# wzjin2017/fhe-fed

Measured on AMD Instinct MI355X. Metric: ciphertexts aggregated/sec (+ encode+enc / dec+decode ms), N clients, ring 2^15 L=4, higher is better.
Workload: dtype u64; 1 GPU; cfg3: 16 learners/GPU x ResNet-18 (11689512 params -> 714 cts of 16384 slots), ring 2^15, L=4 towers; ring_dim=32768, towers=4, learners_total=16, cts_per_learner=714, parallelism=dp1 (one GPU, no collective), layout=arena

## Files before the change

### fhe-fed_amd/csrc/eval.cpp

```cpp
#include <algorithm>
#include <cstring>
#include <fstream>
#include <sstream>

#include "api_util.h"
#include "palisade_codec.h"
#include "shelfi_internal.h"

namespace shelfi {

constexpr int kMaxDigits = 3;

struct LevelState {
  bool built = false;
  bool q_built = false;
  bool own_q = false;
  DeviceTables q;
  DeviceTables ext;
  DeviceTables dtf[kMaxDigits];
  uint64_t* ks = nullptr;
  KsArgs args{};
};

struct EvalState {
// ... 299 lines not shown
  K.T = p.L + ev.kP;
  K.dnum = ev.dnum;
  for (uint32_t t = 0; t < K.T; ++t) {
    K.q.push_back(t < p.L ? p.q[t] : ev.p[t - p.L]);
    K.psi.push_back(t < p.L ? p.psi[t] : ev.ppsi[t - p.L]);
  }
  for (auto& v : K.poly_versions) v = 0;
  return K;
}

static std::string slurp(const std::string& path) {
  std::ifstream f(path, std::ios::binary);
  if (!f) throw Error{SHELFI_ERR_IO, "cannot read " + path};
  std::ostringstream ss;
  ss << f.rdbuf();
  return ss.str();
}

static void load_evalkey(shelfi_ctx* ctx, const std::string& file) {
  EvalState& ev = eval_state(ctx);
  const PalisadeEvalKey K = palisade_parse_evalmult_key((const uint8_t*)file.data(), file.size());
  const Params& p = ctx->p;
  if (ctx->pal_keytag.empty() || K.keytag != ctx->pal_keytag)
    throw Error{SHELFI_ERR_FORMAT, "evaluation key belongs to another key pair (key tag)"};
  if (K.N != p.N || K.T != p.L + ev.kP || K.dnum != ev.dnum)
    throw Error{SHELFI_ERR_FORMAT, "evaluation key was made for other parameters"};
  for (uint32_t t = 0; t < K.T; ++t)
    if (K.q[t] != (t < p.L ? p.q[t] : ev.p[t - p.L]))
      throw Error{SHELFI_ERR_FORMAT, "evaluation key towers differ from this context's Q and special primes"};
  if (K.tower_off.size() != 2ull * K.dnum * K.T) throw Error{SHELFI_ERR_FORMAT, "evaluation key tower count"};
  for (uint32_t t = 0; t < K.T; ++t)
    if (K.psi[t] != (t < p.L ? p.psi[t] : ev.ppsi[t - p.L]))
      throw Error{SHELFI_ERR_FORMAT, "evaluation key roots of unity differ from this context's"};
  std::vector<uint64_t> polys(K.tower_off.size() * (size_t)K.N);
  for (size_t i = 0; i < K.tower_off.size(); ++i)
    std::memcpy(polys.data() + i * K.N, file.data() + K.tower_off[i], (size_t)K.N * 8);
  install_evk(ctx, ev, polys.data());
}

void load_evalkey_if_present(shelfi_ctx* ctx, const std::string& dir) {
  std::string file;
  try {
    file = slurp(dir + "key-eval-mult.txt");
  } catch (const Error&) {
    return;
  }
  try {
    load_evalkey(ctx, file);
  } catch (const Error&) {
  }
}

static uint64_t chunk_of(uint64_t K, size_t per_ct) {
  const uint64_t cap = std::max<uint64_t>(1, (2048ull << 20) / std::max<size_t>(per_ct, 1));
  const uint64_t n = (K + cap - 1) / cap;
  return n ? (K + n - 1) / n : 1;
}

}

using namespace shelfi;

extern "C" {

int shelfi_special_primes(uint32_t ring_dim, uint32_t num_towers, const uint64_t* moduli, uint32_t* dnum,
                          uint32_t* alpha, uint32_t* num_special, uint64_t* special, uint64_t* special_roots) {
  if (!moduli || !dnum || !alpha || !num_special || !special || num_towers < 1 ||
      num_towers > (uint32_t)kMaxTowers || ring_dim < 2 || (ring_dim & (ring_dim - 1)))
    return SHELFI_ERR_ARG;
  return guarded([&] {
    uint64_t p[kMaxTowers], r[kMaxTowers];
    special_primes(ring_dim, num_towers, moduli, dnum, alpha, num_special, p, r);
    for (uint32_t i = 0; i < *num_special; ++i) {
      special[i] = p[i];
      if (special_roots) special_roots[i] = r[i];
    }
  });
}

int shelfi_eval_key_info(const shelfi_ctx* ctx, uint32_t* dnum, uint32_t* alpha, uint32_t* num_special,
                         uint64_t* special, int* has_key) {
  if (!ctx || !dnum || !alpha || !num_special) return SHELFI_ERR_ARG;
  std::lock_guard<std::mutex> lk(ctx->mu);
  return guarded([&] {
    uint64_t p[kMaxTowers];
    special_primes(ctx->p.N, ctx->p.L, ctx->p.q, dnum, alpha, num_special, p, nullptr);
    if (special)
      for (uint32_t i = 0; i < *num_special; ++i) special[i] = p[i];
    if (has_key) *has_key = (ctx->ev && ctx->ev->evk) ? 1 : 0;
  });
}

size_t shelfi_eval_key_words(const shelfi_ctx* ctx) {
  if (!ctx) return 0;
  uint32_t dn, al, kP;
  uint64_t p[kMaxTowers];
  special_primes(ctx->p.N, ctx->p.L, ctx->p.q, &dn, &al, &kP, p, nullptr);
  return 2ull * dn * (ctx->p.L + kP) * ctx->p.N;
}

}

namespace shelfi {
static std::vector<uint64_t> switch_keygen(shelfi_ctx* ctx, uint32_t galois) {
  require_keys(ctx);
  const Params& p = ctx->p;
  EvalState& ev = eval_state(ctx);
// ... 360 lines not shown
```

### fhe-fed_amd/csrc/kernels.hip

```cpp
#include <hip/hip_runtime.h>

#include <algorithm>
#include <cmath>
#include <cstring>
#include <type_traits>
#include <vector>

#include "dev_common.h"
#include "shelfi_internal.h"

namespace shelfi {

static uint32_t xcd_combos(uint64_t G) {
  if (!switches().xcd_order) return 0;
  return (G % 8 == 0 && G <= 0xFFFFFFFFull) ? (uint32_t)G : 0;
}

template <int LOGR>
__global__ __launch_bounds__(256) void ntt_fwd_cols(uint64_t* __restrict__ polys, uint32_t L,
                                                    uint32_t logN, const uint64_t* __restrict__ tw,
                                                    const uint64_t* __restrict__ twp,
                                                    const TowerConst* __restrict__ tcs) {
  constexpr int R = 1 << LOGR;
  const uint32_t N = 1u << logN;
// ... 613 lines not shown
    return (uint32_t)n;
  }();
  uint64_t pc = (uint64_t)cus * per_cu / ncombo;
  if (pc < 1) pc = 1;
  if (pc > K) pc = K;
  return (uint32_t)pc;
}

template <class FZ = NoFuse>
__global__ __launch_bounds__(256) void ntt_inv_blocks(uint64_t* __restrict__ polys, uint32_t L,
                                                      uint32_t logN, uint32_t blkLog,
                                                      const uint64_t* __restrict__ tw,
                                                      const uint64_t* __restrict__ twp,
                                                      const TowerConst* __restrict__ tcs,
                                                      int scale_ninv,
                                                      const uint64_t* __restrict__ ct,
                                                      const uint64_t* __restrict__ sk,
                                                      const uint64_t* __restrict__ sksh, int sum_in,
                                                      uint32_t ctL, FZ fz) {
  constexpr bool FUSE = std::is_same<FZ, FuseIn>::value;
  extern __shared__ __attribute__((aligned(16))) uint64_t sm[];
  const uint32_t N = 1u << logN, blk = 1u << blkLog;
  const uint32_t sh = logN - blkLog, nb = 1u << sh;
  const uint64_t poly = blockIdx.x >> sh;
  const uint32_t b = blockIdx.x & (nb - 1);
  const uint32_t t = (uint32_t)(poly % L);
  const TowerConst& c = tcs[t];
  const uint64_t q = c.q;
  uint64_t* __restrict__ a = polys + poly * N + ((uint64_t)b << blkLog);
  if constexpr (FUSE) {
    const uint64_t e0 = ((poly / L) * ctL << logN) + ((uint64_t)t << logN) + ((uint64_t)b << blkLog);
    for (uint32_t p = threadIdx.x; p < blk / 2; p += 256) {
      ulonglong2 x = make_ulonglong2(0, 0);
      for (uint32_t i = 0; i < fz.P; ++i) {
        const ulonglong2 y = reinterpret_cast<const ulonglong2*>(fz.part[i] + e0)[p];
        x.x += y.x;
        x.y += y.y;
      }
      lds_put2(sm, p, make_ulonglong2(red64(x.x, q, c.one_shoup), red64(x.y, q, c.one_shoup)));
    }
  } else if (ct) {
    const uint64_t kk = poly / L, off = ((uint64_t)t << logN) + ((uint64_t)b << blkLog);
    const ulonglong2* c0 = reinterpret_cast<const ulonglong2*>(ct + (kk * 2 * ctL << logN) + off);
    const ulonglong2* c1 = reinterpret_cast<const ulonglong2*>(ct + ((kk * 2 + 1) * ctL << logN) + off);
    const ulonglong2* s = reinterpret_cast<const ulonglong2*>(sk + off);
    const ulonglong2* ss = reinterpret_cast<const ulonglong2*>(sksh + off);
    for (uint32_t p = threadIdx.x; p < blk / 2; p += 256) {
      ulonglong2 x0 = c0[p];
      const ulonglong2 x1 = c1[p], sv = s[p], sw = ss[p];
      if (sum_in) x0 = make_ulonglong2(red64(x0.x, q, c.one_shoup), red64(x0.y, q, c.one_shoup));
      lds_put2(sm, p, make_ulonglong2(addmod(x0.x, shoup_mul(x1.x, sv.x, sw.x, q), q),
                                      addmod(x0.y, shoup_mul(x1.y, sv.y, sw.y, q), q)));
    }
  } else {
    for (uint32_t p = threadIdx.x; p < blk / 2; p += 256)
      lds_put2(sm, p, reinterpret_cast<const ulonglong2*>(a)[p]);
  }
  __syncthreads();
  ntt_inv_block_stages(sm, blkLog, b, logN, tw + (uint64_t)t * N, twp + (uint64_t)t * N, q);
  if (scale_ninv) {
    const uint64_t ni = c.ninv, nip = c.ninv_shoup;
    for (uint32_t p = threadIdx.x; p < blk / 2; p += 256) {
      const ulonglong2 v = lds_get2(sm, p);
      reinterpret_cast<ulonglong2*>(a)[p] = make_ulonglong2(canon4(shoup_lazy(v.x, ni, nip, q), q),
                                                            canon4(shoup_lazy(v.y, ni, nip, q), q));
    }
  } else {
    for (uint32_t p = threadIdx.x; p < blk / 2; p += 256)
      reinterpret_cast<ulonglong2*>(a)[p] = lds_get2(sm, p);
  }
}

template <int LOGR>
__global__ __launch_bounds__(256) void ntt_inv_cols(uint64_t* __restrict__ polys, uint32_t L,
                                                    uint32_t logN, const uint64_t* __restrict__ tw,
                                                    const uint64_t* __restrict__ twp,
                                                    const TowerConst* __restrict__ tcs) {
  constexpr int R = 1 << LOGR;
  const uint32_t N = 1u << logN;
  const uint32_t BLK = N >> LOGR;
  const uint32_t bpp = BLK / 256;
  const uint64_t poly = blockIdx.x / bpp;
  const uint32_t col = (blockIdx.x % bpp) * 256 + threadIdx.x;
  const uint32_t t = (uint32_t)(poly % L);
  const TowerConst& c = tcs[t];
  const uint64_t q = c.q;
  const uint64_t* __restrict__ w = tw + (uint64_t)t * N;
  const uint64_t* __restrict__ wp = twp + (uint64_t)t * N;
  uint64_t* __restrict__ a = polys + poly * N + col;
  uint64_t x[R];
#pragma unroll
  for (int r = 0; r < R; ++r) x[r] = a[(uint64_t)r * BLK];
#pragma unroll
  for (int v = 0; v < LOGR; ++v) {
    const int tr = 1 << v, h = R >> (v + 1);
#pragma unroll
    for (int i = 0; i < h; ++i) {
      const uint64_t W = w[h + i], Wp = wp[h + i];
#pragma unroll
      for (int jj = 0; jj < tr; ++jj) {
        const int r0 = 2 * i * tr + jj, r1 = r0 + tr;
        if (gs_in8<true>(v, jj))
          gs_bfly_b<true>(x[r0], x[r1], W, Wp, q, c.n8q);
        else
          gs_bfly_b<false>(x[r0], x[r1], W, Wp, q, c.n8q);
      }
    }
  }
  const uint64_t ni = c.ninv, nip = c.ninv_shoup;
#pragma unroll
  for (int r = 0; r < R; ++r) a[(uint64_t)r * BLK] = canon4(shoup_lazy(x[r], ni, nip, q), q);
}

#define NTT_DISPATCH(LOGRV, KERNEL, ...)                                                   \
  switch (LOGRV) {                                                                       \
    case 1: hipLaunchKernelGGL(KERNEL<1>, __VA_ARGS__); break;                           \
    case 2: hipLaunchKernelGGL(KERNEL<2>, __VA_ARGS__); break;                           \
    case 3: hipLaunchKernelGGL(KERNEL<3>, __VA_ARGS__); break;                           \
    case 4: hipLaunchKernelGGL(KERNEL<4>, __VA_ARGS__); break;                           \
    case 5: hipLaunchKernelGGL(KERNEL<5>, __VA_ARGS__); break;                           \
    case 6: hipLaunchKernelGGL(KERNEL<6>, __VA_ARGS__); break;                           \
    default: throw Error{SHELFI_ERR_ARG, "unsupported ring dimension"};                  \
  }

template <int BL, int K1, int K2, int K3, int K4>
__global__ __launch_bounds__(256) void ntt_fwd_blocks_ct(uint64_t* polys, uint32_t L, uint32_t logN,
                                                         const ulonglong2* __restrict__ twb,
                                                         const TowerConst* __restrict__ tcs) {
  __shared__ __attribute__((aligned(16))) uint64_t sm[lpad_size(BL)];
  const uint32_t sh = logN - BL;
  const uint64_t poly = blockIdx.x >> sh;
  const uint32_t b = blockIdx.x & ((1u << sh) - 1);
  const uint32_t t = (uint32_t)(poly % L);
  const TowerConst& c = tcs[t];
  uint64_t* base = polys + (poly << logN) + ((uint64_t)b << BL);
  fwd_block_pass_ct<BL, K1, K2, K3, K4>(base, twb + ((uint64_t)t << logN) + ((uint64_t)b << BL), c.q, c.n8q, sm,
                                        [&](uint32_t j0, auto& x) {
#pragma unroll
                                          for (int m = 0; m < (1 << K4); m += 2)
                                            *reinterpret_cast<ulonglong2*>(base + j0 + m) =
                                                make_ulonglong2(red_any(x[m], c), red_any(x[m + 1], c));
                                        });
}
template <int BL, int K1, int K2, int K3, int K4>
__global__ __launch_bounds__(256) void ntt_inv_blocks_ct(uint64_t* polys, uint32_t L, uint32_t logN,
                                                         const ulonglong2* __restrict__ twb,
                                                         const TowerConst* __restrict__ tcs) {
  static_assert(K1 + K2 + K3 + K4 == BL, "chunk plan must cover the block");
  __shared__ __attribute__((aligned(16))) uint64_t sm[lpad_size(BL)];
  const uint32_t sh = logN - BL;
  const uint64_t poly = blockIdx.x >> sh;
  const uint32_t b = blockIdx.x & ((1u << sh) - 1);
  const uint32_t t = (uint32_t)(poly % L);
  const uint64_t q = tcs[t].q, n8q = tcs[t].n8q;
  uint64_t* base = polys + (poly << logN) + ((uint64_t)b << BL);
  const ulonglong2* __restrict__ tb = twb + ((uint64_t)t << logN) + ((uint64_t)b << BL);
  const auto lds_ld = [&](uint32_t, uint32_t pj) { return sm[pj]; };
  inv_chunk_ct<BL, 0, K1, false>(tb, q, n8q, [&](uint32_t j, uint32_t) { return base[j]; },
                                 [&](int, uint32_t, uint32_t pj0, auto& x) {
#pragma unroll
                                   for (int m = 0; m < (1 << K1); ++m) sm[pj0 + lofs<1>(m)] = x[m];
                                 });
  __syncthreads();
  inv_chunk_ct<BL, K1, K2, true>(tb, q, n8q, lds_ld, [&](int, uint32_t, uint32_t pj0, auto& x) {
#pragma unroll
    for (int m = 0; m < (1 << K2); ++m) sm[pj0 + lofs<(1 << K1)>(m)] = x[m];
  });
  __syncthreads();
  inv_chunk_ct<BL, K1 + K2, K3, true>(tb, q, n8q, lds_ld, [&](int, uint32_t, uint32_t pj0, auto& x) {
#pragma unroll
    for (int m = 0; m < (1 << K3); ++m) sm[pj0 + lofs<(1 << (K1 + K2))>(m)] = x[m];
  });
  __syncthreads();
  inv_chunk_ct<BL, BL - K4, K4, true>(tb, q, n8q, lds_ld, [&](int, uint32_t j0, uint32_t, auto& x) {
#pragma unroll
    for (int m = 0; m < (1 << K4); ++m) base[j0 + (m << (BL - K4))] = x[m];
  });
}

void launch_ntt(uint64_t* polys, uint64_t P, uint32_t L, uint32_t logN, bool inverse,
                const DeviceTables& dt, hipStream_t s) {
  if (!P) return;
  const uint32_t N = 1u << logN;
  const uint32_t blkLog = ntt_block_log(logN);
  const int logR = (int)(logN - blkLog);
  const uint32_t blk = 1u << blkLog;
  const size_t lds = (size_t)blk * sizeof(uint64_t);
  const uint64_t nbBlocks = P << logR;
  const uint64_t nbCols = P * ((N >> logR) / 256);
  if (nbBlocks > 0x7FFFFFFFull || nbCols > 0x7FFFFFFFull)
    throw Error{SHELFI_ERR_ARG, "NTT batch too large"};
  if (!inverse) {
    if (logR > 0) {
      NTT_DISPATCH(logR, ntt_fwd_cols, dim3((uint32_t)nbCols), dim3(256), 0, s, polys, L, logN,
                   dt.psi_rev, dt.psi_rev_sh, dt.tc);
    }
    if (logR > 0 && blkLog == 11 && dt.red_ok)
      hipLaunchKernelGGL((ntt_fwd_blocks_ct<11, 3, 3, 3, 2>), dim3((uint32_t)nbBlocks), dim3(256), 0, s, polys, L,
                         logN, dt.tw_fwd_blk, dt.tc);
    else if (logR > 0 && blkLog == 12 && dt.red_ok)
      hipLaunchKernelGGL((ntt_fwd_blocks_ct<12, 3, 3, 3, 3>), dim3((uint32_t)nbBlocks), dim3(256), 0, s, polys, L,
                         logN, dt.tw_fwd_blk, dt.tc);
    else
      hipLaunchKernelGGL(ntt_fwd_blocks, dim3((uint32_t)nbBlocks), dim3(256), lds, s, polys, L,
                         logN, (uint32_t)logR, dt.psi_rev, dt.psi_rev_sh, dt.tc);
  } else {
    if (logR > 0 && blkLog == 11 && dt.red_ok)
      hipLaunchKernelGGL((ntt_inv_blocks_ct<11, 2, 3, 3, 3>), dim3((uint32_t)nbBlocks), dim3(256), 0, s, polys, L,
                         logN, dt.tw_inv_blk, dt.tc);
    else if (logR > 0 && blkLog == 12 && dt.red_ok)
      hipLaunchKernelGGL((ntt_inv_blocks_ct<12, 3, 3, 3, 3>), dim3((uint32_t)nbBlocks), dim3(256), 0, s, polys, L,
                         logN, dt.tw_inv_blk, dt.tc);
    else
      hipLaunchKernelGGL(ntt_inv_blocks<>, dim3((uint32_t)nbBlocks), dim3(256), lds, s, polys, L,
                         logN, blkLog, dt.ipsi_rev, dt.ipsi_rev_sh, dt.tc, logR == 0 ? 1 : 0,
                         (const uint64_t*)nullptr, (const uint64_t*)nullptr, (const uint64_t*)nullptr, 0, L,
                         NoFuse{});
    if (logR > 0) {
      NTT_DISPATCH(logR, ntt_inv_cols, dim3((uint32_t)nbCols), dim3(256), 0, s, polys, L, logN,
                   dt.ipsi_rev, dt.ipsi_rev_sh, dt.tc);
    }
  }
  SHELFI_HIP(hipGetLastError());
}

void launch_ntt_cols(uint64_t* polys, uint64_t P, uint32_t L, uint32_t logN, bool inverse,
                     const DeviceTables& dt, hipStream_t s) {
  const uint32_t N = 1u << logN;
  const int logR = (int)(logN - ntt_block_log(logN));
  if (!P || logR == 0) return;
  const uint64_t nbCols = P * ((N >> logR) / 256);
  if (nbCols > 0x7FFFFFFFull) throw Error{SHELFI_ERR_ARG, "NTT batch too large"};
  if (!inverse)
    NTT_DISPATCH(logR, ntt_fwd_cols, dim3((uint32_t)nbCols), dim3(256), 0, s, polys, L, logN, dt.psi_rev,
                 dt.psi_rev_sh, dt.tc)
  else
    NTT_DISPATCH(logR, ntt_inv_cols, dim3((uint32_t)nbCols), dim3(256), 0, s, polys, L, logN, dt.ipsi_rev,
                 dt.ipsi_rev_sh, dt.tc)
  SHELFI_HIP(hipGetLastError());
}

template <int LOGR>
__global__ __launch_bounds__(256) void fft_inv_cols(const double* __restrict__ x, uint64_t n,
                                                    double2* __restrict__ buf, uint32_t logS,
                                                    const double2* __restrict__ tw) {
  constexpr int R = 1 << LOGR;
  const uint32_t S = 1u << logS;
  const uint32_t BLK = S >> LOGR;
  const uint32_t bpp = BLK / 256;
  const uint64_t k = blockIdx.x / bpp;
  const uint32_t col = (blockIdx.x % bpp) * 256 + threadIdx.x;
  double2 v[R];
#pragma unroll
  for (int r = 0; r < R; ++r) {
    const uint64_t gi = k * S + col + (uint64_t)r * BLK;
    v[r] = make_double2(gi < n ? x[gi] : 0.0, 0.0);
  }
#pragma unroll
  for (int s = 0; s < LOGR; ++s) {
    const uint32_t len = S >> s, lenh = len >> 1;
    const int trr = R >> (s + 1);
#pragma unroll
    for (int r0 = 0; r0 < R; ++r0) {
      if ((r0 / trr) % 2) continue;
      const int r1 = r0 + trr;
      const uint32_t j = col + (uint32_t)(r0 & ((R >> s) - 1)) * BLK;
      const double2 W = tw[lenh + j];
      const double2 u = cadd(v[r0], v[r1]);
      const double2 d = csub(v[r0], v[r1]);
      v[r0] = u;
      v[r1] = cmul(d, W);
    }
  }
#pragma unroll
  for (int r = 0; r < R; ++r) buf[k * S + col + (uint64_t)r * BLK] = v[r];
}

__global__ __launch_bounds__(256) void fft_inv_blocks(const double* __restrict__ x, uint64_t n,
                                                      double2* __restrict__ buf, uint32_t logS,
                                                      uint32_t blkLog, int from_x,
                                                      const double2* __restrict__ tw) {
  extern __shared__ __attribute__((aligned(16))) double2 smc[];
  const uint32_t S = 1u << logS, blk = 1u << blkLog;
  const uint32_t sh = logS - blkLog;
  const uint64_t k = blockIdx.x >> sh;
  const uint32_t b = blockIdx.x & ((1u << sh) - 1);
  const uint64_t off = k * S + ((uint64_t)b << blkLog);
  for (uint32_t i = threadIdx.x; i < blk; i += 256) {
    if (from_x) {
      const uint64_t gi = off + i;
      smc[i] = make_double2(gi < n ? x[gi] : 0.0, 0.0);
// ... 1956 lines not shown
```

### fhe-fed_amd/csrc/keyswitch.hip

```cpp
#include <hip/hip_runtime.h>

#include <algorithm>

#include "dev_common.h"
#include "shelfi_internal.h"

namespace shelfi {

typedef unsigned __int128 du128;

#define NTT_DISPATCH_KS(LOGRV, KERNEL, ...)                                               \
  switch (LOGRV) {                                                                       \
    case 1: hipLaunchKernelGGL(KERNEL<1>, __VA_ARGS__); break;                           \
    case 2: hipLaunchKernelGGL(KERNEL<2>, __VA_ARGS__); break;                           \
    case 3: hipLaunchKernelGGL(KERNEL<3>, __VA_ARGS__); break;                           \
    case 4: hipLaunchKernelGGL(KERNEL<4>, __VA_ARGS__); break;                           \
    case 5: hipLaunchKernelGGL(KERNEL<5>, __VA_ARGS__); break;                           \
    case 6: hipLaunchKernelGGL(KERNEL<6>, __VA_ARGS__); break;                           \
    default: throw Error{SHELFI_ERR_ARG, "EvalMult: unsupported ring dimension"};        \
  }

__device__ __forceinline__ uint64_t red128(du128 acc, const TowerConst& c) {
  const uint64_t hi = (uint64_t)(acc >> 64), lo = (uint64_t)acc;
  return addmod(shoup_mul(hi, c.r64, c.r64_shoup, c.q), red64(lo, c.q, c.one_shoup), c.q);
// ... 477 lines not shown
    hipLaunchKernelGGL((ks_inner_blocks_ct<11, 3, 3, 3, 2>), grid(K * a.T, nb), dim3(256),
                       sizeof(uint64_t) * lpad_size(11) * a.dn, s, d2e, ext, K, a, dte.tw_fwd_blk, evk, evk_sh, accQ,
                       accP);
  } else {
    if (lds * a.dn > 65536)
      SHELFI_HIP(hipFuncSetAttribute(reinterpret_cast<const void*>(&ks_inner_blocks_kernel),
                                     hipFuncAttributeMaxDynamicSharedMemorySize, (int)(lds * a.dn)));
    hipLaunchKernelGGL(ks_inner_blocks_kernel, grid(K * a.T, nb), dim3(256), lds * a.dn, s, d2e, ext, K, a, blkLog,
                       dte.psi_rev, dte.psi_rev_sh, evk, evk_sh, accQ, accP);
  }
  SHELFI_HIP(hipGetLastError());
  launch_ntt(accP, K * 2 * a.kP, a.kP, a.logN, true, tower_view(dte, a.Ll, N), s);
  if (fuse_cols) {
    NTT_DISPATCH_KS(logR, moddown_cols_kernel, grid(K * 2, (uint32_t)((N >> logR) / 256)), dim3(256), 0, s, accP, a,
                    dtq.psi_rev, dtq.psi_rev_sh, z);
  } else {
    hipLaunchKernelGGL(moddown_kernel, grid(K * 2, bpr), dim3(256), 0, s, accP, a, z);
    SHELFI_HIP(hipGetLastError());
    launch_ntt_cols(z, K * 2 * a.Ll, a.Ll, a.logN, false, dtq, s);
  }
  SHELFI_HIP(hipGetLastError());
  if (sh > 0 && blkLog == 11 && dtq.red_ok)
    hipLaunchKernelGGL((ks_finish_blocks_ct<11, 3, 3, 3, 2>), grid(K * 2 * a.Ll, nb), dim3(256), 0, s, z, accQ, a,
                       dtq.tw_fwd_blk, out);
  else if (sh > 0 && blkLog == 12 && dtq.red_ok)
    hipLaunchKernelGGL((ks_finish_blocks_ct<12, 3, 3, 3, 3>), grid(K * 2 * a.Ll, nb), dim3(256), 0, s, z, accQ, a,
                       dtq.tw_fwd_blk, out);
  else
    hipLaunchKernelGGL(ks_finish_blocks_kernel, grid(K * 2 * a.Ll, nb), dim3(256), lds, s, z, accQ, a, blkLog,
                       dtq.psi_rev, dtq.psi_rev_sh, out);
  SHELFI_HIP(hipGetLastError());
}

__global__ __launch_bounds__(256) void rescale_lift_kernel(const uint64_t* __restrict__ last, uint32_t Lo,
                                                           uint32_t logN, uint64_t ql,
                                                           const TowerConst* __restrict__ tq,
                                                           uint64_t* __restrict__ v) {
  const uint32_t N = 1u << logN, bpr = N >> 8;
  const uint64_t row = blockIdx.x / bpr;
  const uint32_t n = (blockIdx.x % bpr) * 256 + threadIdx.x;
  const uint32_t t = (uint32_t)(row % Lo);
  const TowerConst c = tq[t];
  const uint64_t x = last[(row / Lo) * N + n];
  uint64_t r;
  if (x > (ql >> 1)) {
    const uint64_t m = red64(ql - x, c.q, c.one_shoup);
    r = m ? c.q - m : 0;
  } else {
    r = red64(x, c.q, c.one_shoup);
  }
  v[row * N + n] = r;
}

__global__ __launch_bounds__(256) void rescale_finish_blocks_kernel(const uint64_t* __restrict__ in,
                                                                    const uint64_t* __restrict__ v, uint32_t Lo,
                                                                    uint32_t logN, uint32_t blkLog,
                                                                    const uint64_t* __restrict__ tw,
                                                                    const uint64_t* __restrict__ twp,
                                                                    const TowerConst* __restrict__ tq,
                                                                    RescaleConst rc, uint64_t* __restrict__ out) {
  extern __shared__ __attribute__((aligned(16))) uint64_t sm[];
  const uint32_t N = 1u << logN, blk = 1u << blkLog, sh = logN - blkLog;
  const uint64_t row = blockIdx.x >> sh;
  const uint32_t b = blockIdx.x & ((1u << sh) - 1);
  const uint64_t kp = row / Lo;
  const uint32_t t = (uint32_t)(row % Lo);
  const uint64_t q = tq[t].q, w = rc.qlinv[t], wp = rc.qlinv_sh[t];
  const uint64_t boff = (uint64_t)b << blkLog;
  const ulonglong2* V = reinterpret_cast<const ulonglong2*>(v + (row << logN) + boff);
  for (uint32_t p = threadIdx.x; p < blk / 2; p += 256) lds_put2(sm, p, V[p]);
  __syncthreads();
  ntt_fwd_block_stages(sm, blkLog, b, logN, tw + (uint64_t)t * N, twp + (uint64_t)t * N, q);
  const ulonglong2* X = reinterpret_cast<const ulonglong2*>(in + ((kp * (Lo + 1) + t) << logN) + boff);
  ulonglong2* O = reinterpret_cast<ulonglong2*>(out + (row << logN) + boff);
  for (uint32_t p = threadIdx.x; p < blk / 2; p += 256) {
    const ulonglong2 y = lds_get2(sm, p), x = X[p];
    O[p] = make_ulonglong2(shoup_mul(submod(x.x, canon8(y.x, q), q), w, wp, q),
                           shoup_mul(submod(x.y, canon8(y.y, q), q), w, wp, q));
  }
}

size_t rescale_scratch_bytes(uint32_t Ll, uint32_t N, uint64_t K) {
  return K * 2ull * N * 8 * (1 + (uint64_t)(Ll - 1)) + 64;
}

template <int BL, int K1, int K2, int K3, int K4>
__global__ __launch_bounds__(256) void rescale_finish_blocks_ct(const uint64_t* __restrict__ in,
                                                                const uint64_t* __restrict__ v, uint32_t Lo,
                                                                uint32_t logN, const ulonglong2* __restrict__ twb,
                                                                const TowerConst* __restrict__ tq, RescaleConst rc,
                                                                uint64_t* __restrict__ out) {
  __shared__ __attribute__((aligned(16))) uint64_t sm[lpad_size(BL)];
  const uint32_t sh = logN - BL;
  const uint64_t row = blockIdx.x >> sh;
  const uint32_t b = blockIdx.x & ((1u << sh) - 1);
  const uint64_t kp = row / Lo;
  const uint32_t t = (uint32_t)(row % Lo);
  const TowerConst& c = tq[t];
  const uint64_t q = c.q, w = rc.qlinv[t], wp = rc.qlinv_sh[t];
  const uint64_t boff = (uint64_t)b << BL;
  const ulonglong2* __restrict__ tb = twb + ((uint64_t)t << logN) + boff;
  const uint64_t* __restrict__ X = in + ((kp * (Lo + 1) + t) << logN) + boff;
  uint64_t* __restrict__ O = out + (row << logN) + boff;
  fwd_block_pass_ct<BL, K1, K2, K3, K4>(v + (row << logN) + boff, tb, q, c.n8q, sm, [&](uint32_t j0, auto& y) {
#pragma unroll
    for (int m = 0; m < (1 << K4); m += 2) {
      const ulonglong2 x = *reinterpret_cast<const ulonglong2*>(X + j0 + m);
      *reinterpret_cast<ulonglong2*>(O + j0 + m) =
          make_ulonglong2(shoup_mul(submod(x.x, red_any(y[m], c), q), w, wp, q),
                          shoup_mul(submod(x.y, red_any(y[m + 1], c), q), w, wp, q));
    }
  });
}

void launch_rescale(const DeviceTables& dt, uint32_t Ll, uint32_t logN, const RescaleConst& rc,
                    const uint64_t* in, uint64_t K, uint64_t* out, void* scratch, hipStream_t s) {
  if (!K) return;
  const uint32_t N = 1u << logN, bpr = N >> 8, Lo = Ll - 1;
  uint64_t* last = reinterpret_cast<uint64_t*>(scratch);
  uint64_t* v = last + K * 2 * N;
  SHELFI_HIP(hipMemcpy2DAsync(last, (size_t)N * 8, in + (uint64_t)Lo * N, (size_t)Ll * N * 8, (size_t)N * 8,
                              K * 2, hipMemcpyDeviceToDevice, s));
  launch_ntt(last, K * 2, 1, logN, true, tower_view(dt, Lo, N), s);
  const uint64_t rows = K * 2 * Lo;
  if (rows * bpr > 0x7FFFFFFFull) throw Error{SHELFI_ERR_ARG, "ModReduce batch too large"};
  hipLaunchKernelGGL(rescale_lift_kernel, dim3((uint32_t)(rows * bpr)), dim3(256), 0, s, last, Lo, logN, rc.ql,
                     dt.tc, v);
  SHELFI_HIP(hipGetLastError());
  launch_ntt_cols(v, rows, Lo, logN, false, dt, s);
  const uint32_t blkLog = ntt_block_log(logN);
  const dim3 nbf((uint32_t)(rows << (logN - blkLog)));
  if (logN > blkLog && blkLog == 11 && dt.red_ok)
    hipLaunchKernelGGL((rescale_finish_blocks_ct<11, 3, 3, 3, 2>), nbf, dim3(256), 0, s, in, v, Lo, logN,
                       dt.tw_fwd_blk, dt.tc, rc, out);
  else if (logN > blkLog && blkLog == 12 && dt.red_ok)
    hipLaunchKernelGGL((rescale_finish_blocks_ct<12, 3, 3, 3, 3>), nbf, dim3(256), 0, s, in, v, Lo, logN,
                       dt.tw_fwd_blk, dt.tc, rc, out);
  else
    hipLaunchKernelGGL(rescale_finish_blocks_kernel, nbf, dim3(256), sizeof(uint64_t) << blkLog, s, in, v, Lo,
                       logN, blkLog, dt.psi_rev, dt.psi_rev_sh, dt.tc, rc, out);
  SHELFI_HIP(hipGetLastError());
}

__global__ __launch_bounds__(256) void evk_sample_kernel(uint32_t logN, uint32_t T0,
                                                         const TowerConst* __restrict__ te,
                                                         const uint64_t* __restrict__ cdt, int T, Key8 key,
                                                         uint64_t nonce_base, uint32_t j,
                                                         uint64_t* __restrict__ e_out,
                                                         uint64_t* __restrict__ a_out) {
  const uint32_t N = 1u << logN;
  const uint32_t gid = blockIdx.x * 256 + threadIdx.x;
  if (gid >= (N >> 3)) return;
  const uint32_t j0 = gid * 8;
  const uint64_t nonce = nonce_base | ((uint64_t)j << 16);
  uint64_t re[8];
  chacha20_block(key, j0 >> 3, nonce, re);
  int64_t ev[8];
#pragma unroll
  for (int u = 0; u < 8; ++u) ev[u] = gauss_sample(re[u], cdt, T);
  for (uint32_t t = 0; t < T0; ++t) {
    const TowerConst c = te[t];
    uint64_t ra[16];
    chacha20_block(key, j0 >> 2, nonce | (1 + t), ra);
    chacha20_block(key, (j0 >> 2) + 1, nonce | (1 + t), ra + 8);
#pragma unroll
    for (int u = 0; u < 8; ++u) {
      e_out[(uint64_t)t * N + j0 + u] = mod_signed_dev(ev[u], c);
      const uint64_t lo = ra[2 * u], hi = ra[2 * u + 1];
      a_out[(uint64_t)t * N + j0 + u] =
          addmod(shoup_mul(red64(hi, c.q, c.one_shoup), c.r64, c.r64_shoup, c.q), red64(lo, c.q, c.one_shoup),
                 c.q);
    }
  }
}

__global__ __launch_bounds__(256) void evk_s_ext_kernel(const uint64_t* __restrict__ s0, uint64_t q0,
                                                        uint32_t logN, uint32_t kP,
                                                        const TowerConst* __restrict__ tp,
                                                        uint64_t* __restrict__ sp) {
  const uint32_t N = 1u << logN;
  const uint64_t e = (uint64_t)blockIdx.x * 256 + threadIdx.x;
  if (e >= (uint64_t)kP * N) return;
  const uint32_t m = (uint32_t)(e >> logN);
// ... 71 lines not shown
```

### fhe-fed_amd/csrc/shelfi_internal.h

```cpp
#pragma once

#include <hip/hip_runtime.h>

#include <cstdint>
#include <cstdlib>
#include <mutex>
#include <string>
#include <vector>

#include "../../include/shelfi.h"

namespace shelfi {

typedef unsigned __int128 u128;

void set_error(const std::string& msg);
struct Error {
  int code;
  std::string msg;
};
#define SHELFI_HIP(expr)                                                             \
  do {                                                                               \
    hipError_t _e = (expr);                                                          \
    if (_e != hipSuccess)                                                            \
      throw ::shelfi::Error{SHELFI_ERR_DEVICE, std::string(#expr) + ": " +           \
                                                 hipGetErrorString(_e)};             \
  } while (0)

constexpr int kMaxTowers = 16;
constexpr int kMaxCommRanks = 16;
constexpr int kFftBlockLog = 10;
constexpr int kFftBlockLogBig = 11;
inline uint32_t fft_block_log(uint32_t logS) {
  const uint32_t b = logS >= 15 ? (uint32_t)kFftBlockLogBig : (uint32_t)kFftBlockLog;
  return logS < b ? logS : b;
}
constexpr int kNttBlockLog = 11;
constexpr int kNttBlockLogBig = 12;
inline uint32_t ntt_block_log(uint32_t logN) {
  static const uint32_t ovr = [] {
    const char* e = std::getenv("SHELFI_NTT_BLOCK_LOG_BIG");
    const int v = e ? std::atoi(e) : 0;
    return (uint32_t)((v == 11 || v == 12) ? v : 0);
  }();
  uint32_t b = logN >= 17 ? (uint32_t)kNttBlockLogBig : (uint32_t)kNttBlockLog;
  if (ovr && logN >= 16) b = ovr;
  return logN < b ? logN : b;
}

struct Switches {
  bool xcd_order = true;
  bool ntt_wl = true;
  bool fft_ct = true;
  bool fft_whole = true;
  bool enc_fused = true;
  bool enc_pp = true;
  bool dec_pp = true;
  bool enc_nored = true;
  bool enc_tab = true;
  bool enc_vt = true;
  int enc_ts = -1;
  bool dec_all_towers = false;
  bool stage_trace = false;
  bool enc_x5 = true;
  int pack_kernel = 0;
  int pack_unroll = 0;
  int pack_waves = 0;
  int wavg_rows = 0;
  uint32_t wavg_strands = 0;
  int arena_stager = -1;
  uint64_t dev_chunk_mib = 4096;
  uint64_t wavg_chunk_mib = 0;
  uint64_t stage_slot_mib = 16;
  bool h2d_direct = false;
  bool h2d_two = true;
};
const Switches& switches();
void reload_switches();

struct Params {
  uint32_t N = 0, logN = 0, L = 0, batch = 0, gap = 0, scale_bits = 0, first_mod_bits = 0;
  uint64_t q[kMaxTowers] = {0};
  uint64_t psi[kMaxTowers] = {0};
  double delta = 0.0;
  double sigma = 3.19;
};

uint64_t powmod(uint64_t a, uint64_t e, uint64_t q);
uint64_t invmod(uint64_t a, uint64_t q);
uint64_t shoup(uint64_t w, uint64_t q);
uint64_t mod_signed(int64_t v, uint64_t q);
bool is_prime(uint64_t n);
uint32_t default_ring_dim(uint32_t L, uint32_t scale_bits, uint32_t first_mod_bits, uint32_t batch);
uint32_t hybrid_dnum(uint32_t L);
double ring_dim_qbound(uint32_t L, uint32_t scale_bits, uint32_t first_mod_bits);
void generate_chain(uint32_t N, uint32_t L, uint32_t scale_bits, uint32_t first_mod_bits,
                    uint64_t* q, uint64_t* psi);
uint64_t min_root(uint64_t m, uint64_t q);
void special_primes(uint32_t N, uint32_t L, const uint64_t* q, uint32_t* dnum, uint32_t* alpha,
                    uint32_t* kP, uint64_t* p, uint64_t* ppsi);
void fft_twiddles(uint32_t slots, double* inv_re, double* inv_im, double* fwd_re, double* fwd_im);
int gauss_cdt(double sigma, uint64_t* cdt, int max_entries);
uint64_t fnv1a(const void* data, size_t n, uint64_t h = 1469598103934665603ull);

struct TowerConst {
  uint64_t q;
  uint64_t one_shoup;
  uint64_t r30, r30_shoup;
  uint64_t r60, r60_shoup;
  uint64_t r64, r64_shoup;
  uint64_t ninv, ninv_shoup;
  uint64_t qhat_inv, qhat_inv_shoup;
  double inv_q;
  uint64_t nq, n4q, n8q;
  uint32_t red_r, red_sh, red_ok;
  uint32_t crt_sh;
  float inv_q32;
  uint32_t pad32;
  uint64_t bq62;
  uint64_t ninv_qhat, ninv_qhat_shoup;
  uint64_t ninv_qhat_w1, ninv_qhat_w1_shoup;
  uint32_t crt30[7], nq30[7];
  uint64_t crt_edge[2];
};

constexpr int kEncVTab = 4 * 81, kEncETab = 128, kEncTab = kEncVTab + kEncETab;

struct DeviceTables {
// ... 104 lines not shown
  void* io = nullptr;
  size_t io_bytes = 0;
  uint64_t* gather_host = nullptr;
  size_t gather_cap = 0;
  shelfi::EvalState* ev = nullptr;
  void* comm = nullptr;
  int comm_rank = 0, comm_world = 0;
  hipStream_t comm_stream = nullptr;
  std::vector<hipEvent_t> comm_events;
};

namespace shelfi {

constexpr int kWavgMaxLearners = 16;
constexpr int kArenaChunk = 512;
struct WavgArgs {
  const uint64_t* ptrs[kWavgMaxLearners];
  uint32_t wl[kWavgMaxLearners][kMaxTowers][2];
  uint64_t* out;
  uint64_t rows;
  uint32_t C, L, logN, accumulate;
  uint32_t* bad;
};
void launch_wavg(const WavgArgs& a, const TowerConst* tc, hipStream_t s);
struct ArenaPack {
  uint32_t w[kMaxTowers];
  uint32_t pre[kMaxTowers];
  uint32_t sum;
};
ArenaPack arena_pack(const Params& p);
uint64_t arena_ct_words(const Params& p, uint64_t C);
void launch_wavg_packed(const uint64_t* arena, const uint32_t* wl_dev, uint32_t C, uint64_t rows, uint32_t L,
                        uint32_t logN, const ArenaPack& ap, const TowerConst* tc, uint64_t* out, hipStream_t s);
void launch_wavg_packed_ex(const uint32_t* in, const uint32_t* wl_dev, uint32_t C, uint32_t crow, uint64_t lstride,
                           uint64_t rows, uint32_t L, uint32_t logN, const ArenaPack& ap, const TowerConst* tc,
                           uint64_t* out, uint32_t* pout, hipStream_t s);
void launch_arena_pack(const uint64_t* src, uint64_t row0, uint64_t rows, uint32_t C, uint32_t learner,
                       uint32_t L, uint32_t logN, const ArenaPack& ap, const TowerConst* tc, uint64_t* arena,
                       uint32_t* bad, hipStream_t s);
void launch_blob_pack(const uint64_t* src, uint64_t K, uint32_t L, uint32_t logN, const ArenaPack& ap,
                      const TowerConst* tc, uint32_t* dst, uint32_t* bad, hipStream_t s);
void launch_blob_unpack(const uint32_t* src, uint64_t K, uint32_t L, uint32_t logN, const ArenaPack& ap,
                        uint64_t* dst, hipStream_t s);
void launch_gather_runs(const uint8_t* raw, const uint64_t* src_off, uint64_t runs, uint32_t run_bytes, uint8_t* dst,
                        hipStream_t s);
void launch_modq(uint64_t* buf, uint64_t rows, uint32_t L, uint32_t logN, const TowerConst* tc,
                 hipStream_t s);
void launch_check_residues(const uint64_t* ct, uint64_t rows, uint32_t L, uint32_t logN, const TowerConst* tc,
                           uint32_t* bad, hipStream_t s);
void launch_ntt(uint64_t* polys, uint64_t P, uint32_t L, uint32_t logN, bool inverse,
                const DeviceTables& dt, hipStream_t s);
void launch_ntt_cols(uint64_t* polys, uint64_t P, uint32_t L, uint32_t logN, bool inverse,
                     const DeviceTables& dt, hipStream_t s);
struct GenFlag {
  uint32_t* p = nullptr;
  uint32_t gen = 0;
};
void launch_encrypt(const Params& p, const DeviceTables& dt, const DeviceKeys& dk,
                    const double* x, uint64_t n, uint64_t K, uint64_t* ct, void* scratch,
                    const uint32_t key[8], uint64_t g0, GenFlag flag, hipStream_t s);
void launch_encrypt_approx(const Params& p, const DeviceTables& dt, const DeviceKeys& dk, const double* x,
                           uint64_t n, uint64_t K, uint64_t* ct, void* scratch, const uint32_t key[8],
                           uint64_t g0, hipStream_t s);
size_t encrypt_scratch_bytes(const Params& p, uint64_t K);
struct DecodeNoise {
  int enabled = 0;
  double m_factor = 1.0;
  uint32_t p_bits = 52;
  uint32_t key[8] = {};
  uint64_t g0 = 0;
  uint32_t* flags = nullptr;
  GenFlag fail;
  int reset = 1;
};
struct FuseIn {
  const uint64_t* part[kMaxCommRanks];
  uint32_t P;
};
struct NoFuse {};
void launch_decrypt(const Params& p, const DeviceTables& dt, const DeviceKeys& dk,
                    const uint64_t* ct, uint64_t K, double scale, uint64_t n, double* out,
                    void* scratch, hipStream_t s, const DecodeNoise* dn = nullptr, bool sum_in = false,
                    uint32_t ct_L = 0,
                    GenFlag crt_flag = GenFlag{}, bool exact = false,
                    const FuseIn* fuse_in = nullptr);
size_t decrypt_scratch_bytes(const Params& p, uint64_t K);
void launch_keygen(const Params& p, const DeviceTables& dt, const uint32_t key[8], uint64_t* sk,
                   uint64_t* pk, void* scratch, hipStream_t s);
size_t keygen_scratch_bytes(const Params& p);
void launch_keygen_chain(const Params& p, const DeviceTables& dt, const uint32_t key[8], const uint64_t* prev_pk,
                         uint64_t* sk, uint64_t* pk, void* scratch, hipStream_t s);
size_t keygen_chain_scratch_bytes(const Params& p);
size_t partial_decrypt_scratch_bytes(const Params& p, uint32_t towers, uint64_t K, double sigma);
void launch_partial_decrypt(const Params& p, const DeviceTables& dt, const DeviceKeys& dk, const uint64_t* ct,
                            uint64_t K, uint32_t towers, bool lead, uint64_t* out, void* scratch, double sigma,
                            const uint32_t key[8], uint64_t g0, hipStream_t s);

void wavg_arena_enqueue(shelfi_ctx* ctx, const uint64_t* arena_dev, const float* w, size_t C, size_t K,
                        uint64_t* out_dev, hipStream_t s);
void wavg_arena_enqueue_packed(shelfi_ctx* ctx, const uint64_t* arena_dev, const float* w, size_t C, size_t K,
                               uint64_t* out_packed, hipStream_t s);
void sum_packed_enqueue(shelfi_ctx* ctx, const uint64_t* stacked, size_t G, size_t K, size_t stride,
                        uint64_t* out, hipStream_t s);
void arena_require_valid_locked(const shelfi_ctx* ctx, const uint64_t* a, size_t words);
void check_wavg_weights(const float* w, size_t C, double delta);
void comm_release(shelfi_ctx* ctx);
void eval_release(shelfi_ctx* ctx, bool keys_only);
void load_evalkey_if_present(shelfi_ctx* ctx, const std::string& dir);
const DeviceTables& level_tables(shelfi_ctx* ctx, uint32_t Ll);
void seed_to_key(uint64_t seed, uint32_t key[8]);
void os_random(void* buf, size_t n);
void require_keys(const shelfi_ctx* ctx);

struct KsArgs {
  uint32_t Ll, kP, T, dn, alpha, logN, Lfull, dnFull;
  const uint64_t* mu_inv;
  const uint64_t* mu_inv_sh;
  const uint64_t* mu_hat;
  const uint64_t* md_inv;
  const uint64_t* md_inv_sh;
  const uint64_t* md_hat;
  const uint64_t* pinv;
  const uint64_t* pinv_sh;
  const TowerConst* tq;
  const TowerConst* te;
};
size_t ks_scratch_bytes(uint32_t Ll, uint32_t kP, uint32_t dn, uint32_t alpha, uint32_t N, uint64_t K);
void launch_eval_mult(const KsArgs& a, const DeviceTables& dtq, const DeviceTables& dte,
                      const DeviceTables* dtf, const uint64_t* evk, const uint64_t* evk_sh, const uint64_t* x,
                      const uint64_t* y, uint64_t K, uint64_t* out, void* scratch, hipStream_t s);
struct KsScratch {
  uint64_t *d2e, *d2c, *ext, *accQ, *accP, *z;
// ... 29 lines not shown
```

### fhe-fed_amd/csrc/switches.cpp

```cpp
#include <atomic>
#include <cstdlib>
#include <cstring>
#include <initializer_list>

#include "shelfi_internal.h"

namespace shelfi {

static std::atomic<const Switches*> g_switches{nullptr};

static bool env_flag(const char* name, char off_or_on, bool dflt) {
  const char* e = getenv(name);
  return e && *e == off_or_on ? !dflt : dflt;
}
static int env_choice(const char* name, std::initializer_list<int> allowed, int dflt) {
  const char* e = getenv(name);
  if (!e) return dflt;
  const int v = atoi(e);
  for (int a : allowed)
    if (a == v) return v;
  return dflt;
}

void reload_switches() {
  Switches s;
  s.xcd_order = env_flag("SHELFI_XCD_ORDER", '0', true);
  s.ntt_wl = env_flag("SHELFI_NTT_WL", '0', true);
  s.fft_ct = env_flag("SHELFI_FFT_CT", '0', true);
  s.fft_whole = env_flag("SHELFI_FFT_WHOLE", '0', true);
  s.enc_fused = env_flag("SHELFI_ENC_FUSED_COLS", '0', true);
  s.enc_pp = env_flag("SHELFI_ENC_PP", '0', true);
  s.dec_pp = env_flag("SHELFI_DEC_PP", '0', true);
  s.enc_nored = env_flag("SHELFI_ENC_NORED", '0', true);
  s.enc_tab = env_flag("SHELFI_ENC_TAB", '0', true);
  s.enc_vt = env_flag("SHELFI_ENC_VT", '0', true);
  s.enc_ts = env_choice("SHELFI_ENC_TS", {0, 1}, -1);
  s.dec_all_towers = env_flag("SHELFI_DEC_ALL_TOWERS", '1', false);
  s.enc_x5 = env_flag("SHELFI_ENC_X5", '0', true);
  s.stage_trace = env_choice("SHELFI_STAGE_TRACE", {0, 1}, 0) == 1;
  if (const char* e = getenv("SHELFI_PACK_KERNEL")) s.pack_kernel = !strcmp(e, "v4") ? 4 : !strcmp(e, "r3") ? 3 : 0;
  s.pack_unroll = env_choice("SHELFI_PACK_UNROLL", {1, 2, 4, 8}, 0);
  s.pack_waves = env_choice("SHELFI_PACK_WAVES", {2, 8}, 0);
  s.wavg_rows = env_choice("SHELFI_WAVG_ROWS", {1, 2}, 0);
  if (const char* e = getenv("SHELFI_WAVG_STRANDS"))
    if (atoi(e) > 1 && atoi(e) <= 4096) s.wavg_strands = (uint32_t)atoi(e);
  s.arena_stager = env_choice("SHELFI_ARENA_STAGER", {0, 1}, -1);
  if (const char* e = getenv("SHELFI_DEV_CHUNK_MIB"))
    if (atoll(e) > 0) s.dev_chunk_mib = (uint64_t)atoll(e);
  if (const char* e = getenv("SHELFI_WAVG_CHUNK_MIB"))
    if (atoll(e) > 0) s.wavg_chunk_mib = (uint64_t)atoll(e);
  if (const char* e = getenv("SHELFI_STAGE_SLOT_MIB"))
    if (atoll(e) > 0 && atoll(e) <= 256) s.stage_slot_mib = (uint64_t)atoll(e);
  s.h2d_direct = env_flag("SHELFI_H2D_DIRECT", '1', false);
  s.h2d_two = env_flag("SHELFI_H2D_TWO", '0', true);
  g_switches.store(new Switches(s), std::memory_order_release);
}
const Switches& switches() { return *g_switches.load(std::memory_order_acquire); }
static const bool g_switches_read = (reload_switches(), true);

}

extern "C" {

void shelfi_reload_switches(void) { shelfi::reload_switches(); }

}
```

Baseline: 3.372 million client-ciphertexts/s.

## Fuse rescale gather, inverse NTT and lift into fewer kernels

The rescale (ModReduce) path no longer copies the last tower into scratch with a 2D memcpy. The inverse NTT block pass now reads it directly from the pitched ciphertext. A new column kernel then finishes the inverse NTT column stages, does the centered lift into each remaining tower, and runs the forward NTT column stages in registers, replacing three separate launches and their round trips through global memory. The eval chunk budget is also tied to the dev_chunk_mib switch. The new path adds register pressure from holding R values across all towers, and the work is serialised over towers inside each thread.

```diff
diff --git a/fhe-fed_amd/csrc/eval.cpp b/fhe-fed_amd/csrc/eval.cpp
--- a/fhe-fed_amd/csrc/eval.cpp
+++ b/fhe-fed_amd/csrc/eval.cpp
@@ -375,7 +375,8 @@
 }
 
 static uint64_t chunk_of(uint64_t K, size_t per_ct) {
-  const uint64_t cap = std::max<uint64_t>(1, (2048ull << 20) / std::max<size_t>(per_ct, 1));
+  const uint64_t budget = std::min<uint64_t>(2048, switches().dev_chunk_mib) << 20;
+  const uint64_t cap = std::max<uint64_t>(1, budget / std::max<size_t>(per_ct, 1));
   const uint64_t n = (K + cap - 1) / cap;
   return n ? (K + n - 1) / n : 1;
 }
diff --git a/fhe-fed_amd/csrc/kernels.hip b/fhe-fed_amd/csrc/kernels.hip
--- a/fhe-fed_amd/csrc/kernels.hip
+++ b/fhe-fed_amd/csrc/kernels.hip
@@ -689,6 +689,9 @@
       lds_put2(sm, p, make_ulonglong2(addmod(x0.x, shoup_mul(x1.x, sv.x, sw.x, q), q),
                                       addmod(x0.y, shoup_mul(x1.y, sv.y, sw.y, q), q)));
     }
+  } else if constexpr (std::is_same<FZ, PitchedIn>::value) {
+    const ulonglong2* src = reinterpret_cast<const ulonglong2*>(fz.src + poly * fz.pitch + ((uint64_t)b << blkLog));
+    for (uint32_t p = threadIdx.x; p < blk / 2; p += 256) lds_put2(sm, p, src[p]);
   } else {
     for (uint32_t p = threadIdx.x; p < blk / 2; p += 256)
       lds_put2(sm, p, reinterpret_cast<const ulonglong2*>(a)[p]);
@@ -779,10 +782,10 @@
                                                 make_ulonglong2(red_any(x[m], c), red_any(x[m + 1], c));
                                         });
 }
-template <int BL, int K1, int K2, int K3, int K4>
+template <int BL, int K1, int K2, int K3, int K4, class SRC = NoFuse>
 __global__ __launch_bounds__(256) void ntt_inv_blocks_ct(uint64_t* polys, uint32_t L, uint32_t logN,
                                                          const ulonglong2* __restrict__ twb,
-                                                         const TowerConst* __restrict__ tcs) {
+                                                         const TowerConst* __restrict__ tcs, SRC src) {
   static_assert(K1 + K2 + K3 + K4 == BL, "chunk plan must cover the block");
   __shared__ __attribute__((aligned(16))) uint64_t sm[lpad_size(BL)];
   const uint32_t sh = logN - BL;
@@ -792,8 +795,10 @@
   const uint64_t q = tcs[t].q, n8q = tcs[t].n8q;
   uint64_t* base = polys + (poly << logN) + ((uint64_t)b << BL);
   const ulonglong2* __restrict__ tb = twb + ((uint64_t)t << logN) + ((uint64_t)b << BL);
+  const uint64_t* in = base;
+  if constexpr (std::is_same<SRC, PitchedIn>::value) in = src.src + poly * src.pitch + ((uint64_t)b << BL);
   const auto lds_ld = [&](uint32_t, uint32_t pj) { return sm[pj]; };
-  inv_chunk_ct<BL, 0, K1, false>(tb, q, n8q, [&](uint32_t j, uint32_t) { return base[j]; },
+  inv_chunk_ct<BL, 0, K1, false>(tb, q, n8q, [&](uint32_t j, uint32_t) { return in[j]; },
                                  [&](int, uint32_t, uint32_t pj0, auto& x) {
 #pragma unroll
                                    for (int m = 0; m < (1 << K1); ++m) sm[pj0 + lofs<1>(m)] = x[m];
@@ -844,10 +849,10 @@
   } else {
     if (logR > 0 && blkLog == 11 && dt.red_ok)
       hipLaunchKernelGGL((ntt_inv_blocks_ct<11, 2, 3, 3, 3>), dim3((uint32_t)nbBlocks), dim3(256), 0, s, polys, L,
-                         logN, dt.tw_inv_blk, dt.tc);
+                         logN, dt.tw_inv_blk, dt.tc, NoFuse{});
     else if (logR > 0 && blkLog == 12 && dt.red_ok)
       hipLaunchKernelGGL((ntt_inv_blocks_ct<12, 3, 3, 3, 3>), dim3((uint32_t)nbBlocks), dim3(256), 0, s, polys, L,
-                         logN, dt.tw_inv_blk, dt.tc);
+                         logN, dt.tw_inv_blk, dt.tc, NoFuse{});
     else
       hipLaunchKernelGGL(ntt_inv_blocks<>, dim3((uint32_t)nbBlocks), dim3(256), lds, s, polys, L,
                          logN, blkLog, dt.ipsi_rev, dt.ipsi_rev_sh, dt.tc, logR == 0 ? 1 : 0,
@@ -874,6 +879,27 @@
   else
     NTT_DISPATCH(logR, ntt_inv_cols, dim3((uint32_t)nbCols), dim3(256), 0, s, polys, L, logN, dt.ipsi_rev,
                  dt.ipsi_rev_sh, dt.tc)
+  SHELFI_HIP(hipGetLastError());
+}
+
+void launch_ntt_inv_blocks_from(const uint64_t* src, uint64_t src_pitch, uint64_t* dst, uint64_t P, uint32_t logN,
+                                const DeviceTables& dt, hipStream_t s) {
+  if (!P) return;
+  const uint32_t blkLog = ntt_block_log(logN);
+  const int logR = (int)(logN - blkLog);
+  const uint64_t nbBlocks = P << logR;
+  if (nbBlocks > 0x7FFFFFFFull) throw Error{SHELFI_ERR_ARG, "NTT batch too large"};
+  const PitchedIn pin{src, src_pitch};
+  if (logR > 0 && blkLog == 11 && dt.red_ok)
+    hipLaunchKernelGGL((ntt_inv_blocks_ct<11, 2, 3, 3, 3, PitchedIn>), dim3((uint32_t)nbBlocks), dim3(256), 0, s, dst,
+                       1u, logN, dt.tw_inv_blk, dt.tc, pin);
+  else if (logR > 0 && blkLog == 12 && dt.red_ok)
+    hipLaunchKernelGGL((ntt_inv_blocks_ct<12, 3, 3, 3, 3, PitchedIn>), dim3((uint32_t)nbBlocks), dim3(256), 0, s, dst,
+                       1u, logN, dt.tw_inv_blk, dt.tc, pin);
+  else
+    hipLaunchKernelGGL(ntt_inv_blocks<PitchedIn>, dim3((uint32_t)nbBlocks), dim3(256), sizeof(uint64_t) << blkLog, s,
+                       dst, 1u, logN, blkLog, dt.ipsi_rev, dt.ipsi_rev_sh, dt.tc, logR == 0 ? 1 : 0,
+                       (const uint64_t*)nullptr, (const uint64_t*)nullptr, (const uint64_t*)nullptr, 0, 1u, pin);
   SHELFI_HIP(hipGetLastError());
 }
 
diff --git a/fhe-fed_amd/csrc/keyswitch.hip b/fhe-fed_amd/csrc/keyswitch.hip
--- a/fhe-fed_amd/csrc/keyswitch.hip
+++ b/fhe-fed_amd/csrc/keyswitch.hip
@@ -553,6 +553,82 @@
   v[row * N + n] = r;
 }
 
+template <int LOGR>
+__global__ __launch_bounds__(256) void rescale_cols_kernel(const uint64_t* __restrict__ last, uint32_t Lo,
+                                                           uint32_t logN, uint64_t ql,
+                                                           const TowerConst* __restrict__ tq,
+                                                           const uint64_t* __restrict__ itw,
+                                                           const uint64_t* __restrict__ itwp,
+                                                           const uint64_t* __restrict__ tw,
+                                                           const uint64_t* __restrict__ twp,
+                                                           uint64_t* __restrict__ v) {
+  constexpr int R = 1 << LOGR;
+  const uint32_t N = 1u << logN, BLK = N >> LOGR, bpp = BLK / 256;
+  const uint64_t row = blockIdx.x / bpp;
+  const uint32_t col = (blockIdx.x % bpp) * 256 + threadIdx.x;
+  uint64_t c[R];
+  uint32_t neg = 0;
+  {
+    const TowerConst& cl = tq[Lo];
+    const uint64_t q = cl.q;
+    const uint64_t* __restrict__ a = last + (row << logN) + col;
+#pragma unroll
+    for (int r = 0; r < R; ++r) c[r] = a[(uint64_t)r * BLK];
+#pragma unroll
+    for (int st = 0; st < LOGR; ++st) {
+      const int tr = 1 << st, h = R >> (st + 1);
+#pragma unroll
+      for (int i = 0; i < h; ++i) {
+        const uint64_t W = itw[h + i], Wp = itwp[h + i];
+#pragma unroll
+        for (int jj = 0; jj < tr; ++jj) {
+          const int r0 = 2 * i * tr + jj, r1 = r0 + tr;
+          if (gs_in8<true>(st, jj))
+            gs_bfly_b<true>(c[r0], c[r1], W, Wp, q, cl.n8q);
+          else
+            gs_bfly_b<false>(c[r0], c[r1], W, Wp, q, cl.n8q);
+        }
+      }
+    }
+    const uint64_t ni = cl.ninv, nip = cl.ninv_shoup, half = ql >> 1;
+#pragma unroll
+    for (int r = 0; r < R; ++r) {
+      const uint64_t x = canon4(shoup_lazy(c[r], ni, nip, q), q);
+      const bool ng = x > half;
+      c[r] = ng ? ql - x : x;
+      neg |= (uint32_t)ng << r;
+    }
+  }
+  for (uint32_t t = 0; t < Lo; ++t) {
+    const TowerConst& ct = tq[t];
+    const uint64_t q = ct.q, os = ct.one_shoup;
+    uint64_t x[R];
+#pragma unroll
+    for (int r = 0; r < R; ++r) {
+      const uint64_t m = red64(c[r], q, os);
+      x[r] = ((neg >> r) & 1) && m ? q - m : m;
+    }
+    const uint64_t* __restrict__ w = tw + (uint64_t)t * N;
+    const uint64_t* __restrict__ wp = twp + (uint64_t)t * N;
+#pragma unroll
+    for (int st = 0; st < LOGR; ++st) {
+      const int m = 1 << st, tr = R >> (st + 1);
+#pragma unroll
+      for (int i = 0; i < m; ++i) {
+        const uint64_t W = w[m + i], Wp = wp[m + i];
+#pragma unroll
+        for (int jj = 0; jj < tr; ++jj) {
+          const int r0 = 2 * i * tr + jj, r1 = r0 + tr;
+          ct_bfly(x[r0], x[r1], W, Wp, q);
+        }
+      }
+    }
+    uint64_t* __restrict__ o = v + ((row * Lo + t) << logN) + col;
+#pragma unroll
+    for (int r = 0; r < R; ++r) o[(uint64_t)r * BLK] = x[r];
+  }
+}
+
 __global__ __launch_bounds__(256) void rescale_finish_blocks_kernel(const uint64_t* __restrict__ in,
                                                                     const uint64_t* __restrict__ v, uint32_t Lo,
                                                                     uint32_t logN, uint32_t blkLog,
@@ -620,16 +696,39 @@
   const uint32_t N = 1u << logN, bpr = N >> 8, Lo = Ll - 1;
   uint64_t* last = reinterpret_cast<uint64_t*>(scratch);
   uint64_t* v = last + K * 2 * N;
-  SHELFI_HIP(hipMemcpy2DAsync(last, (size_t)N * 8, in + (uint64_t)Lo * N, (size_t)Ll * N * 8, (size_t)N * 8,
-                              K * 2, hipMemcpyDeviceToDevice, s));
-  launch_ntt(last, K * 2, 1, logN, true, tower_view(dt, Lo, N), s);
   const uint64_t rows = K * 2 * Lo;
   if (rows * bpr > 0x7FFFFFFFull) throw Error{SHELFI_ERR_ARG, "ModReduce batch too large"};
-  hipLaunchKernelGGL(rescale_lift_kernel, dim3((uint32_t)(rows * bpr)), dim3(256), 0, s, last, Lo, logN, rc.ql,
-                     dt.tc, v);
+  const uint32_t blkLog = ntt_block_log(logN);
+  const int logR = (int)(logN - blkLog);
+  const DeviceTables dtl = tower_view(dt, Lo, N);
+  const bool fused = switches().rescale_fused;
+  if (fused) {
+    launch_ntt_inv_blocks_from(in + (uint64_t)Lo * N, (uint64_t)Ll * N, last, K * 2, logN, dtl, s);
+  } else {
+    SHELFI_HIP(hipMemcpy2DAsync(last, (size_t)N * 8, in + (uint64_t)Lo * N, (size_t)Ll * N * 8, (size_t)N * 8,
+                                K * 2, hipMemcpyDeviceToDevice, s));
+    launch_ntt(last, K * 2, 1, logN, true, dtl, s);
+  }
+  if (fused && logR > 0 && logR <= 4) {
+    const dim3 nbc((uint32_t)(K * 2 * ((N >> logR) / 256)));
+#define RESCALE_COLS(LR)                                                                                         \
+  hipLaunchKernelGGL(rescale_cols_kernel<LR>, nbc, dim3(256), 0, s, last, Lo, logN, rc.ql, dt.tc, dtl.ipsi_rev, \
+                     dtl.ipsi_rev_sh, dt.psi_rev, dt.psi_rev_sh, v)
+    switch (logR) {
+      case 1: RESCALE_COLS(1); break;
+      case 2: RESCALE_COLS(2); break;
+      case 3: RESCALE_COLS(3); break;
+      default: RESCALE_COLS(4); break;
+    }
+#undef RESCALE_COLS
+  } else {
+    if (fused) launch_ntt_cols(last, K * 2, 1, logN, true, dtl, s);
+    hipLaunchKernelGGL(rescale_lift_kernel, dim3((uint32_t)(rows * bpr)), dim3(256), 0, s, last, Lo, logN, rc.ql,
+                       dt.tc, v);
+    SHELFI_HIP(hipGetLastError());
+    launch_ntt_cols(v, rows, Lo, logN, false, dt, s);
+  }
   SHELFI_HIP(hipGetLastError());
-  launch_ntt_cols(v, rows, Lo, logN, false, dt, s);
-  const uint32_t blkLog = ntt_block_log(logN);
   const dim3 nbf((uint32_t)(rows << (logN - blkLog)));
   if (logN > blkLog && blkLog == 11 && dt.red_ok)
     hipLaunchKernelGGL((rescale_finish_blocks_ct<11, 3, 3, 3, 2>), nbf, dim3(256), 0, s, in, v, Lo, logN,
diff --git a/fhe-fed_amd/csrc/shelfi_internal.h b/fhe-fed_amd/csrc/shelfi_internal.h
--- a/fhe-fed_amd/csrc/shelfi_internal.h
+++ b/fhe-fed_amd/csrc/shelfi_internal.h
@@ -74,6 +74,7 @@
   uint64_t stage_slot_mib = 16;
   bool h2d_direct = false;
   bool h2d_two = true;
+  bool rescale_fused = true;
 };
 const Switches& switches();
 void reload_switches();
@@ -284,6 +285,8 @@
                 const DeviceTables& dt, hipStream_t s);
 void launch_ntt_cols(uint64_t* polys, uint64_t P, uint32_t L, uint32_t logN, bool inverse,
                      const DeviceTables& dt, hipStream_t s);
+void launch_ntt_inv_blocks_from(const uint64_t* src, uint64_t src_pitch, uint64_t* dst, uint64_t P, uint32_t logN,
+                                const DeviceTables& dt, hipStream_t s);
 struct GenFlag {
   uint32_t* p = nullptr;
   uint32_t gen = 0;
@@ -310,6 +313,10 @@
   uint32_t P;
 };
 struct NoFuse {};
+struct PitchedIn {
+  const uint64_t* src;
+  uint64_t pitch;
+};
 void launch_decrypt(const Params& p, const DeviceTables& dt, const DeviceKeys& dk,
                     const uint64_t* ct, uint64_t K, double scale, uint64_t n, double* out,
                     void* scratch, hipStream_t s, const DecodeNoise* dn = nullptr, bool sum_in = false,
diff --git a/fhe-fed_amd/csrc/switches.cpp b/fhe-fed_amd/csrc/switches.cpp
--- a/fhe-fed_amd/csrc/switches.cpp
+++ b/fhe-fed_amd/csrc/switches.cpp
@@ -53,6 +53,7 @@
     if (atoll(e) > 0 && atoll(e) <= 256) s.stage_slot_mib = (uint64_t)atoll(e);
   s.h2d_direct = env_flag("SHELFI_H2D_DIRECT", '1', false);
   s.h2d_two = env_flag("SHELFI_H2D_TWO", '0', true);
+  s.rescale_fused = env_flag("SHELFI_RESCALE_FUSED", '0', true);
   g_switches.store(new Switches(s), std::memory_order_release);
 }
 const Switches& switches() { return *g_switches.load(std::memory_order_acquire); }
```

Result: no change. 3.354 million client-ciphertexts/s (-0.5%).
